# ccchengff/SketchML

Hardware: AMD Instinct MI355X
Metric: device-resident grad encode GB/s (fp32 in) + decode L2 err, 1/2/4/8 GPU (higher is better)
Workload: dtype f32; 1 GPU; north star: 2^28-float dense gradient bucket per GPU, 256 requested bins, encode; n_per_gpu=268435456, bins=256, rotating_buffers=2, parallelism=dp1

## Files before the change

### sketchml_amd/csrc/skml_device.hpp

```cpp
#pragma once
#include <hip/hip_runtime.h>
#include <stdint.h>

#include <type_traits>

#include "skml_internal.h"

namespace skml {

__device__ __forceinline__ uint32_t f2key(uint32_t b) {
    return b ^ ((uint32_t)((int32_t)b >> 31) | 0x80000000u);
}
__device__ __forceinline__ uint32_t key2f(uint32_t k) {
    return k ^ ((k >> 31) ? 0x80000000u : 0xFFFFFFFFu);
}
__device__ __forceinline__ bool is_nan_bits(uint32_t b) { return (b & 0x7FFFFFFFu) > 0x7F800000u; }

typedef _Float16 f16x2_v __attribute__((ext_vector_type(2)));
typedef __bf16 bf16x2_v __attribute__((ext_vector_type(2)));
typedef uint32_t u32x4_v __attribute__((ext_vector_type(4)));
template <typename X>
struct is_lowp : std::integral_constant<bool, std::is_same<X, bf16_t>::value || std::is_same<X, f16_t>::value> {};

template <typename X>
// ... 76 lines not shown
    const uint64_t b = (uint64_t)__double_as_longlong(v);
    const uint32_t lo = lane_xor<M>((uint32_t)b), hi = lane_xor<M>((uint32_t)(b >> 32));
    return __longlong_as_double((long long)(((uint64_t)hi << 32) | lo));
}

__device__ __forceinline__ uint32_t wave_incl_scan_u32(uint32_t v) {
    int x = (int)v;
    x += __builtin_amdgcn_update_dpp(0, x, 0x111, 0xF, 0xF, true);
    x += __builtin_amdgcn_update_dpp(0, x, 0x112, 0xF, 0xF, true);
    x += __builtin_amdgcn_update_dpp(0, x, 0x114, 0xF, 0xF, true);
    x += __builtin_amdgcn_update_dpp(0, x, 0x118, 0xF, 0xF, true);
    x += __builtin_amdgcn_update_dpp(0, x, 0x142, 0xA, 0xF, false);
    x += __builtin_amdgcn_update_dpp(0, x, 0x143, 0xC, 0xF, false);
    return (uint32_t)x;
}

template <int OP>
__device__ __forceinline__ uint32_t dpp_op(uint32_t a, uint32_t b) {
    return OP == 0 ? (a < b ? a : b) : OP == 1 ? (a > b ? a : b) : (a | b);
}
template <int OP>
__device__ __forceinline__ uint32_t wave_reduce_u32_lane63(uint32_t v) {
    constexpr int id = OP == 0 ? -1 : 0;
    int x = (int)v;
    x = (int)dpp_op<OP>((uint32_t)x, (uint32_t)__builtin_amdgcn_update_dpp(id, x, 0x111, 0xF, 0xF, false));
    x = (int)dpp_op<OP>((uint32_t)x, (uint32_t)__builtin_amdgcn_update_dpp(id, x, 0x112, 0xF, 0xF, false));
    x = (int)dpp_op<OP>((uint32_t)x, (uint32_t)__builtin_amdgcn_update_dpp(id, x, 0x114, 0xF, 0xF, false));
    x = (int)dpp_op<OP>((uint32_t)x, (uint32_t)__builtin_amdgcn_update_dpp(id, x, 0x118, 0xF, 0xF, false));
    x = (int)dpp_op<OP>((uint32_t)x, (uint32_t)__builtin_amdgcn_update_dpp(id, x, 0x142, 0xA, 0xF, false));
    x = (int)dpp_op<OP>((uint32_t)x, (uint32_t)__builtin_amdgcn_update_dpp(id, x, 0x143, 0xC, 0xF, false));
    return (uint32_t)x;
}

__device__ __forceinline__ uint32_t elem_fbits(uint32_t k) { return key2f(k); }
__device__ __forceinline__ uint32_t elem_fbits(float f) { return __float_as_uint(f); }
template <typename T>
__device__ __forceinline__ T elem_of_fbits(uint32_t b);
template <>
__device__ __forceinline__ uint32_t elem_of_fbits<uint32_t>(uint32_t b) { return f2key(b); }
template <>
__device__ __forceinline__ float elem_of_fbits<float>(uint32_t b) { return __uint_as_float(b); }
template <typename T>
__device__ __forceinline__ T sel_of(bool upper);
template <>
__device__ __forceinline__ uint32_t sel_of<uint32_t>(bool upper) { return upper ? 0xFFFFFFFFu : 0u; }
template <>
__device__ __forceinline__ float sel_of<float>(bool upper) {
    return __uint_as_float(upper ? 0x7F800000u : 0xFF800000u);
}
template <>
__device__ __forceinline__ double sel_of<double>(bool upper) {
    return __longlong_as_double(upper ? 0x7FF0000000000000LL : (long long)0xFFF0000000000000ULL);
}

template <typename T>
struct Elem {
    using S = float;
    __device__ static __forceinline__ S to_s(uint32_t k) { return __uint_as_float(key2f(k)); }
    __device__ static __forceinline__ uint32_t from_s(S f) { return f2key(__float_as_uint(f)); }
};
template <>
struct Elem<float> {
    using S = float;
    __device__ static __forceinline__ S to_s(float f) { return f; }
    __device__ static __forceinline__ float from_s(S f) { return f; }
};
template <>
struct Elem<double> {
    using S = double;
    __device__ static __forceinline__ S to_s(double d) { return d; }
    __device__ static __forceinline__ double from_s(S d) { return d; }
};

__device__ __forceinline__ void ce(uint32_t& a, uint32_t& b) {
    uint32_t lo = a < b ? a : b;
    uint32_t hi = a < b ? b : a;
    a = lo;
    b = hi;
}
__device__ __forceinline__ void ce(float& a, float& b) {
    float lo, hi;
    asm("v_min_f32 %0, %1, %2" : "=v"(lo) : "v"(a), "v"(b));
    asm("v_max_f32 %0, %1, %2" : "=v"(hi) : "v"(a), "v"(b));
    a = lo;
    b = hi;
// ... 102 lines not shown

template <int R, typename T>
__device__ __forceinline__ void halfclean_regs(T (&v)[R]) {
#pragma unroll
    for (int d = R >> 1; d >= 1; d >>= 1) {
#pragma unroll
        for (int i = 0; i < R; i++) {
            int j = i ^ d;
            if (j > i) ce(v[i], v[j]);
        }
    }
}

__device__ __forceinline__ uint32_t umed3(uint32_t a, uint32_t b, uint32_t c) {
    return min(max(a, b), max(min(a, b), c));
}
__device__ __forceinline__ uint32_t med3(uint32_t a, uint32_t b, uint32_t c) { return umed3(a, b, c); }
__device__ __forceinline__ float med3(float a, float b, float c) { return __builtin_amdgcn_fmed3f(a, b, c); }
__device__ __forceinline__ double med3(double a, double b, double c) {
    double lo, hi;
    asm("v_min_f64 %0, %1, %2" : "=v"(lo) : "v"(a), "v"(b));
    asm("v_max_f64 %0, %1, %2" : "=v"(hi) : "v"(a), "v"(b));
    return __double_as_longlong(c) > 0 ? hi : lo;
}

#ifndef SKML_FLIP_GROUP
#define SKML_FLIP_GROUP 4
#endif
#ifndef SKML_HALF_GROUP
#define SKML_HALF_GROUP 8
#endif
template <int R, int M, typename T>
__device__ __forceinline__ void flip_lanes(T (&v)[R], int lane) {
    const T sel = sel_of<T>((lane & ((M + 1) >> 1)) != 0);
#pragma unroll
    for (int r = 0; r < R / 2; r++) {
        const T pa = lane_xor<M>(v[R - 1 - r]);
        const T pb = lane_xor<M>(v[r]);
        v[r] = med3(v[r], pa, sel);
        v[R - 1 - r] = med3(v[R - 1 - r], pb, sel);
        if ((r & (SKML_FLIP_GROUP - 1)) == SKML_FLIP_GROUP - 1) __builtin_amdgcn_sched_barrier(0);
    }
}

template <int R, int D, typename T>
__device__ __forceinline__ void halfclean_lanes(T (&v)[R], int lane) {
    const T sel = sel_of<T>((lane & D) != 0);
#pragma unroll
    for (int r = 0; r < R; r++) {
        v[r] = med3(v[r], lane_xor<D>(v[r]), sel);
        if ((r & (SKML_HALF_GROUP - 1)) == SKML_HALF_GROUP - 1) __builtin_amdgcn_sched_barrier(0);
    }
}

template <int R, int D, typename T>
__device__ __forceinline__ void halfclean_lanes_down(T (&v)[R], int lane) {
    if constexpr (D >= 1) {
        halfclean_lanes<R, D>(v, lane);
        halfclean_lanes_down<R, D / 2>(v, lane);
    }
}

template <int R, typename T>
__device__ __forceinline__ void merge_group(T (&v)[R], int lane) {
    constexpr int G = 256 / R;
    flip_lanes<R, G - 1>(v, lane);
    halfclean_lanes_down<R, G / 4>(v, lane);
    halfclean_regs<R>(v);
}

template <int R, int S, typename T>
__device__ __forceinline__ void sort_lanes_from(T (&v)[R], int lane) {
    if constexpr (S <= 256) {
        constexpr int M = S / R - 1;
        flip_lanes<R, M>(v, lane);
        halfclean_lanes_down<R, S / R / 4>(v, lane);
        halfclean_regs<R>(v);
        sort_lanes_from<R, S * 2>(v, lane);
    }
}
template <int R, typename T>
__device__ __forceinline__ void sort_group256(T (&v)[R], int lane) {
    sort_regs<R>(v);
    sort_lanes_from<R, 2 * R>(v, lane);
}

template <int R>
__device__ __forceinline__ void compact_regs(const uint32_t (&v)[R], uint32_t (&w)[R / 2], bool odd) {
    const uint32_t m = odd ? 0xFFFFFFFFu : 0u;
#pragma unroll
    for (int j = 0; j < R / 2; j++) w[j] = (v[2 * j + 1] & m) | (v[2 * j] & ~m);
}

template <int R, typename T>
__device__ __forceinline__ void halfclean_regs_compact(T (&v)[R], T (&w)[R / 2], bool odd) {
#pragma unroll
    for (int d = R >> 1; d >= 2; d >>= 1) {
#pragma unroll
        for (int i = 0; i < R; i++) {
            int j = i ^ d;
            if (j > i) ce(v[i], v[j]);
        }
    }
    const T sel = sel_of<T>(odd);
#pragma unroll
    for (int j = 0; j < R / 2; j++) w[j] = med3(v[2 * j], v[2 * j + 1], sel);
}

template <int R, typename T>
__device__ __forceinline__ void merge_group_compact(T (&v)[R], T (&w)[R / 2], int lane, bool odd) {
    constexpr int G = 256 / R;
    flip_lanes<R, G - 1>(v, lane);
    halfclean_lanes_down<R, G / 4>(v, lane);
    halfclean_regs_compact<R>(v, w, odd);
}

template <int R, int S, typename T>
__device__ __forceinline__ void sort_lanes_upto128(T (&v)[R], int lane) {
    if constexpr (S <= 128) {
        constexpr int M = S / R - 1;
        flip_lanes<R, M>(v, lane);
        halfclean_lanes_down<R, S / R / 4>(v, lane);
        halfclean_regs<R>(v);
        sort_lanes_upto128<R, S * 2>(v, lane);
    }
}
template <int R, typename T>
__device__ __forceinline__ void sort_group256_compact(T (&v)[R], T (&w)[R / 2], int lane, bool odd) {
    sort_regs<R>(v);
    sort_lanes_upto128<R, 2 * R>(v, lane);
    merge_group_compact<R>(v, w, lane, odd);
}

__device__ __forceinline__ uint64_t lcg_jump(const uint64_t* __restrict__ tab, uint64_t s,
                                             uint64_t steps) {
#pragma unroll
    for (int lvl = 0; lvl < 4; lvl++) {
        uint32_t b = (uint32_t)(steps >> (8 * lvl)) & 255u;
        if (b) {
            const uint64_t a = tab[(lvl * 256 + b) * 2];
            const uint64_t c = tab[(lvl * 256 + b) * 2 + 1];
            s = (a * s + c) & kLcgMask;
        }
    }
    return s;
}
__device__ __forceinline__ uint32_t lcg_bit(const uint64_t* __restrict__ tab, uint64_t s0,
                                            uint64_t idx) {
    return (uint32_t)(lcg_jump(tab, s0, idx + 1) >> 47) & 1u;
}
__device__ __forceinline__ uint64_t node_bit_index(uint64_t c, int level) {
    return 2 * c - (uint64_t)__popcll(c) + (uint64_t)level;
}

template <typename S>
__device__ __forceinline__ int count_le(const S* run, S x) {
    int lo = 0;
#pragma unroll
    for (int step = 64; step >= 1; step >>= 1)
        if (run[lo + step - 1] <= x) lo += step;
    return lo + (run[lo] <= x ? 1 : 0) * (lo == 127 ? 1 : 0);
}
template <typename S>
__device__ __forceinline__ int count_lt(const S* run, S x) {
    int lo = 0;
#pragma unroll
    for (int step = 64; step >= 1; step >>= 1)
        if (run[lo + step - 1] < x) lo += step;
    return lo + (run[lo] < x ? 1 : 0) * (lo == 127 ? 1 : 0);
}
__device__ __forceinline__ uint32_t tie_pred(float s, float v, uint32_t tie) {
    return (uint32_t)(s < v) | ((uint32_t)(s == v) & tie);
}
__device__ __forceinline__ uint32_t tie_pred(double s, double v, uint32_t tie) {
    return (uint32_t)(s < v) | ((uint32_t)(s == v) & tie);
}
template <typename S>
__device__ __forceinline__ int rank_in_run_pair(const S* a, const S* b, S v, uint32_t tie_a, uint32_t tie_b,
// ... 128 lines not shown
```

### sketchml_amd/csrc/skml_sketch.hip

```cpp
#include <cstdlib>
#include <cstring>
#include <type_traits>

#include "skml_device.hpp"

namespace skml {

__device__ unsigned long long g_prof[32];
#ifdef SKML_PROF_LEAF
__device__ unsigned long long g_leafprof[4 * 65536];
#endif
#ifdef SKML_PROF_SUMMARY
#define SKML_PROF(k)                                      \
    do {                                                  \
        if (threadIdx.x == 0) g_prof[(k)] = wall_clock64(); \
    } while (0)
#else
#define SKML_PROF(k) \
    do {             \
    } while (0)
#endif

constexpr int kWaveFb = 1536;
template <typename S>
// ... 306 lines not shown
#pragma unroll
            for (int j = 0; j < 8; j++) f[j] = src[j * 8 + (lane & 7)];
#pragma unroll
            for (int j = 0; j < 8; j++) {
                const float e4[4] = {f[j].x, f[j].y, f[j].z, f[j].w};
#pragma unroll
                for (int e = 0; e < 4; e++) {
                    zmask |= __ballot(is_class(e4[e], 0x63));
                    v[j * 4 + e] = e4[e];
                }
            }
        }
        if (PARTIAL) zmask &= __ballot(valid);
        uint32_t rfl = 0;
        if (zmask) {
            uint64_t nz = 0, pz = 0, nan = 0;
#pragma unroll
            for (int r = 0; r < 32; r++) {
                nz |= __ballot(is_class(v[r], 0x20));
                pz |= __ballot(is_class(v[r], 0x40));
                nan |= __ballot(is_class(v[r], 0x03));
            }
            if (PARTIAL) {
                nz &= __ballot(valid);
                pz &= __ballot(valid);
                nan &= __ballot(valid);
            }
            rfl = (nz ? 2u : 0u) | (pz ? 4u : 0u) | (nan ? 1u : 0u);
            fl |= rfl;
        }
        const uint64_t start = node_bit_index((uint64_t)c0, 0);
        uint64_t mask;
        {
            const uint64_t s_start = lcg_jump(tab, s0, start + 1);
            const uint64_t s = lane == 0 ? s_start : ((ta * s_start + tc) & kLcgMask);
            mask = __ballot((s >> 47) & 1ull);
        }
        if constexpr (STAGE == 0) {
#pragma unroll
            for (int r = 0; r < 32; r++) acc ^= fold32(v[r]);
            acc ^= (uint32_t)mask;
            continue;
        }
        neg_any = neg_any || (rfl & 2u);
        pos_any = pos_any || (rfl & 4u);
        const bool exact = STAGE == 2 ? false : (neg_any && pos_any);
        auto bit = [&](int level, int64_t last_chunk) -> uint32_t {
            return (uint32_t)(mask >> (node_bit_index((uint64_t)last_chunk, level) - start)) & 1u;
        };

        E w1[16];
        {
            sort_regs_oddeven<32>(v);
            sort_lanes_upto128<32, 64>(v, lane);
            if (valid) {
                const Key k0 = total_key(v[0]), k31 = total_key(v[31]);
                mn = k0 < mn ? k0 : mn;
                mx = k31 > mx ? k31 : mx;
            }
            merge_group_compact<32>(v, w1, lane, bit(0, chunk) != 0);
        }
        const WaveExport<PARTIAL, E> exp{lane, rem, round * kChunksPerWave, roots};
        exp.template at<16>(0, lane >> 3, w1);
        if constexpr (STAGE == 1) {
#pragma unroll
            for (int r = 0; r < 16; r++) acc ^= fold32(w1[r]);
            continue;
        }
        uint32_t ibits = 0;
// ... 19 lines not shown
        if (!(round & 2)) {
            st4[0] = n4[0];
            st4[1] = n4[1];
            continue;
        }
        E n5[2];
        wave_node_merge(st4, n4, n5, lane, bit(5, c0 + 7), exact, wfb);
        if constexpr (PARTIAL)
            if (((rem >> 5) & 1) && round == 3) store_node<2>(n5, lane, roots + (size_t)5 * kK);
        if (!(round & 4)) {
            st5[0] = n5[0];
            st5[1] = n5[1];
            continue;
        }
        wave_node_merge(st5, n5, top, lane, bit(6, c0 + 7), exact, wfb);
    }
    if constexpr (STAGE <= 2) {
        nodes6[(size_t)tile * 64 + lane] = (E)(acc ^ (uint32_t)mn ^ (uint32_t)mx ^ fl);
        return;
    }
    if constexpr (!PARTIAL) {
        if (ubits && tile < upper_node_count(chunks)) {
            int L = kLeafTopLevel + 1;
            int64_t i = tile;
            while (i >= (chunks >> L)) i -= chunks >> L++;
            const uint64_t c = ((uint64_t)(i + 1) << L) - 1;
            if (lane == 0) ubits[tile] = (uint8_t)lcg_bit(tab, s0, node_bit_index(c, L));
        }
    }
    if constexpr (!PARTIAL) {
        store_node<2>(top, lane, nodes6 + (size_t)tile * kK);
        if (((chunks >> 6) & 1) && tile == ((chunks >> 7) << 1)) store_node<2>(top, lane, roots + (size_t)6 * kK);
    }
#pragma unroll
    for (int off = 32; off >= 1; off >>= 1) {
        const Key omn = __shfl_xor(mn, off, 64);
        const Key omx = __shfl_xor(mx, off, 64);
        const uint32_t ofl = (uint32_t)__shfl_xor((int)fl, off, 64);
        mn = omn < mn ? omn : mn;
        mx = omx > mx ? omx : mx;
        fl |= ofl;
    }
    if (lane == 0) {
        typename LeafTypes<E>::Part p;
        p.min_key = mn;
        p.max_key = mx;
        p.flags = fl;
        if constexpr (std::is_same<E, float>::value) p.flags |= (mn < 0x007FFFFFu || mx > 0xFF800000u) ? 1u : 0u;
        p.pad = 0;
        part[tile] = p;
#ifdef SKML_PROF_LEAF
        if (!PARTIAL && tile < 65536) {
            g_leafprof[4 * tile] = prof_t0;
            g_leafprof[4 * tile + 1] = wall_clock64();
            g_leafprof[4 * tile + 2] = __builtin_amdgcn_s_getreg((4 << 0) | (0 << 6) | (31 << 11));
            g_leafprof[4 * tile + 3] = __builtin_amdgcn_s_getreg((20 << 0) | (0 << 6) | (31 << 11));
        }
#endif
    }
}

template <int STAGE, bool PARTIAL = false, typename E = float, typename X = E>
__global__ __launch_bounds__(256, LeafTypes<E>::kMinWaves) void k_leaf2(
    const X* __restrict__ x, int64_t chunks, uint64_t s0, const uint64_t* __restrict__ tab,
    typename LeafTypes<E>::Part* __restrict__ part, E* __restrict__ nodes6, E* __restrict__ roots, int64_t tile0,
    uint8_t* __restrict__ ubits = nullptr) {
    __shared__ E fb[kLeaf2Waves][kWaveFb];
    const int wave = threadIdx.x >> 6;
    leaf2_wave<STAGE, PARTIAL, E, X>(x, chunks, s0, tab, part, nodes6, roots,
                                  tile0 + (int64_t)blockIdx.x * kLeaf2Waves + wave, ubits, fb[wave]);
}

constexpr int kL64Lanes = 4;
constexpr int kL64Chunks = 64 / kL64Lanes;
constexpr int kL64Rounds = kLeafWaveChunks / kL64Chunks;

#ifndef SKML_LEAF64_WAVES
#define SKML_LEAF64_WAVES 4
#endif
#ifndef SKML_LEAF_MIN3DET
#define SKML_LEAF_MIN3DET 1
#endif
#ifndef SKML_LEAF_SPLIT_BELOW
#define SKML_LEAF_SPLIT_BELOW 3072
#endif
struct Leaf64Shared {
    float fb[kLeaf2Waves][kWaveFb];
    float2 stk[kLeaf2Waves][2][64];
    uint32_t wpart[kLeaf2Waves][4];
};
template <bool SPLIT, typename X = float>
__device__ __forceinline__ void leaf64_tile(const X* __restrict__ x, int64_t chunks, uint64_t s0,
                                            const uint64_t* __restrict__ tab, LeafPartial* __restrict__ part,
                                            float* __restrict__ nodes6, float* __restrict__ roots,
                                            uint8_t* __restrict__ ubits, int64_t tile, Leaf64Shared& L) {
    auto& fb = L.fb;
    auto& stk = L.stk;
    auto& wpart = L.wpart;
    const int wave = threadIdx.x >> 6, lane = threadIdx.x & 63;
    const int64_t c_tile = tile * kLeafWaveChunks;
    if (c_tile >= chunks) return;
#ifdef SKML_PROF_LEAF
    const unsigned long long prof_t0 = wall_clock64();
#endif
    float* wfb = fb[wave];
    uint32_t mn = ~0u, mx = 0, fl = 0u;
    bool neg_any = false, pos_any = false;
    float top[2];
    uint64_t split_mask = 0;
    auto run_round = [&](auto ex, int round) -> bool {
        constexpr bool EX = decltype(ex)::value;
        int ln = lane;
        asm volatile("" : "+v"(ln));
        if constexpr (!SPLIT) set_prio_by_progress(round, kL64Rounds);
            const int64_t c0 = c_tile + round * kL64Chunks;
            const int64_t chunk = c0 + (ln >> 2);
            float v[64];
            uint64_t zmask = 0;
            if constexpr (is_lowp<X>::value) {
                const u32x4_v* src = reinterpret_cast<const u32x4_v*>(x + chunk * kChunk);
                u32x4_v f[8];
#pragma unroll
                for (int j = 0; j < 8; j++) f[j] = src[j * kL64Lanes + (ln & 3)];
#pragma unroll
                for (int j = 0; j < 8; j++) widen8<X>(f[j], v + j * 8);
#if SKML_LEAF_MIN3DET
                float za = __builtin_inff(), zb = __builtin_inff();
#pragma unroll
                for (int j = 0; j < 16; j++) {
                    asm("v_minimum3_f32 %0, |%1|, |%2|, %3" : "=v"(za) : "v"(v[j * 4 + 0]), "v"(v[j * 4 + 1]), "v"(za));
                    asm("v_minimum3_f32 %0, |%1|, |%2|, %3" : "=v"(zb) : "v"(v[j * 4 + 2]), "v"(v[j * 4 + 3]), "v"(zb));
                }
// ... 17 lines not shown
                    asm("v_minimum3_f32 %0, |%1|, |%2|, %3" : "=v"(zb) : "v"(f[j].z), "v"(f[j].w), "v"(zb));
                    v[j * 4 + 0] = f[j].x, v[j * 4 + 1] = f[j].y, v[j * 4 + 2] = f[j].z, v[j * 4 + 3] = f[j].w;
                }
                float zm;
                asm("v_minimum3_f32 %0, %1, %2, %2" : "=v"(zm) : "v"(za), "v"(zb));
                zmask = __ballot(!(zm > 0.0f));
#else
#pragma unroll
                for (int j = 0; j < 16; j++) {
                    const float e4[4] = {f[j].x, f[j].y, f[j].z, f[j].w};
#pragma unroll
                    for (int e = 0; e < 4; e++) {
                        zmask |= __ballot(is_class(e4[e], 0x63));
                        v[j * 4 + e] = e4[e];
                    }
                }
#endif
            }
            uint32_t rfl = 0;
            if (zmask) {
                uint64_t nz = 0, pz = 0, nan = 0;
#pragma unroll
                for (int r = 0; r < 64; r++) {
                    nz |= __ballot(is_class(v[r], 0x20));
                    pz |= __ballot(is_class(v[r], 0x40));
                    nan |= __ballot(is_class(v[r], 0x03));
                }
                rfl = (nz ? 2u : 0u) | (pz ? 4u : 0u) | (nan ? 1u : 0u);
                fl |= rfl;
            }
            const uint64_t start = node_bit_index((uint64_t)c0, 0);
            uint64_t mask;
            {
                const uint64_t ta = tab[ln * 2], tc = tab[ln * 2 + 1];
                const uint64_t s_start = lcg_jump(tab, s0, start + 1);
                const uint64_t s = ln == 0 ? s_start : ((ta * s_start + tc) & kLcgMask);
                mask = __ballot((s >> 47) & 1ull);
            }
            neg_any = neg_any || (rfl & 2u);
            pos_any = pos_any || (rfl & 4u);
            if constexpr (!EX) {
                if (neg_any && pos_any) return false;
            }
            const bool exact = EX;
            auto bit = [&](int level, int d) -> uint32_t {
                return (uint32_t)(mask >> (2 * d - __popc((unsigned)d) + level)) & 1u;
            };
            float w1[32];
            sort_regs_oddeven<64>(v);
            sort_lanes_upto128<64, 128>(v, ln);
            {
                const uint32_t k0 = total_key(v[0]), k63 = total_key(v[63]);
                mn = k0 < mn ? k0 : mn;
                mx = k63 > mx ? k63 : mx;
            }
            merge_group_compact<64>(v, w1, ln, bit(0, ln >> 2) != 0);
            float w2[16], w3[8], w4[4], n4[2];
#ifdef SKML_LEAF_ABLATE_TREE
            for (int q = 0; q < 16; q++) w2[q] = fminf(w1[2 * q], w1[2 * q + 1]);
            for (int q = 0; q < 8; q++) w3[q] = w2[2 * q];
            for (int q = 0; q < 4; q++) w4[q] = w3[2 * q];
            n4[0] = w4[0];
            n4[1] = w4[2];
#else
            wave_level<32>(w1, w2, ln, bit(1, 2 * (ln >> 3) + 1), exact, wfb);
            wave_level<16>(w2, w3, ln, bit(2, 4 * (ln >> 4) + 3), exact, wfb);
            wave_level<8>(w3, w4, ln, bit(3, 8 * (ln >> 5) + 7), exact, wfb);
            wave_level<4>(w4, n4, ln, bit(4, 15), exact, wfb);
#endif
            if constexpr (SPLIT) {
                stk[wave][0][ln] = make_float2(n4[0], n4[1]);
                split_mask = mask;
                return true;
            }
            if (!(round & 1)) {
                stk[wave][0][ln] = make_float2(n4[0], n4[1]);
                return true;
            }
            float n5[2];
            {
                const float2 o = stk[wave][0][ln];
                const float st4[2] = {o.x, o.y};
                wave_node_merge(st4, n4, n5, ln, bit(5, 15), exact, wfb);
            }
            if (!(round & 2)) {
                stk[wave][1][ln] = make_float2(n5[0], n5[1]);
                return true;
            }
            const float2 o = stk[wave][1][ln];
            const float st5[2] = {o.x, o.y};
            wave_node_merge(st5, n5, top, ln, bit(6, 15), exact, wfb);
            return true;
    };
    if constexpr (SPLIT) {
        if (!run_round(std::false_type{}, wave)) run_round(std::true_type{}, wave);
#pragma unroll
        for (int off = 32; off >= 1; off >>= 1) {
            const uint32_t omn = __shfl_xor(mn, off, 64);
            const uint32_t omx = __shfl_xor(mx, off, 64);
            const uint32_t ofl = (uint32_t)__shfl_xor((int)fl, off, 64);
            mn = omn < mn ? omn : mn;
            mx = omx > mx ? omx : mx;
            fl |= ofl;
        }
        if (lane == 0) {
            wpart[wave][0] = mn;
            wpart[wave][1] = mx;
            wpart[wave][2] = fl;
        }
        __syncthreads();
        auto zs = [&](int w) { return wpart[w][2] & 6u; };
        const uint32_t b5 = (uint32_t)(split_mask >> 31) & 1u, b6 = (uint32_t)(split_mask >> 32) & 1u;
        if (wave & 1) {
            const uint32_t z = zs(wave - 1) | zs(wave);
            const float2 o = stk[wave - 1][0][lane], m = stk[wave][0][lane];
            const float A[2] = {o.x, o.y}, B[2] = {m.x, m.y};
            float n5[2];
            wave_node_merge(A, B, n5, lane, b5, z == 6u, wfb);
            stk[wave][1][lane] = make_float2(n5[0], n5[1]);
        }
        __syncthreads();
        if (wave != 3) return;
        {
            const uint32_t z = zs(0) | zs(1) | zs(2) | zs(3);
            const float2 o = stk[1][1][lane], m = stk[3][1][lane];
            const float A[2] = {o.x, o.y}, B[2] = {m.x, m.y};
            wave_node_merge(A, B, top, lane, b6, z == 6u, wfb);
        }
        mn = min(min(wpart[0][0], wpart[1][0]), min(wpart[2][0], wpart[3][0]));
        mx = max(max(wpart[0][1], wpart[1][1]), max(wpart[2][1], wpart[3][1]));
        fl = wpart[0][2] | wpart[1][2] | wpart[2][2] | wpart[3][2];
    } else {
        int round = 0;
#pragma unroll 1
        for (; round < kL64Rounds; round++)
            if (!run_round(std::false_type{}, round)) break;
#pragma unroll 1
        for (; round < kL64Rounds; round++) run_round(std::true_type{}, round);
    }
    if (ubits && tile < upper_node_count(chunks)) {
        int L = kLeafTopLevel + 1;
        int64_t i = tile;
        while (i >= (chunks >> L)) i -= chunks >> L++;
        const uint64_t c = ((uint64_t)(i + 1) << L) - 1;
        if (lane == 0) ubits[tile] = (uint8_t)lcg_bit(tab, s0, node_bit_index(c, L));
    }
    store_node<2>(top, lane, nodes6 + (size_t)tile * kK);
    if (((chunks >> 6) & 1) && tile == ((chunks >> 7) << 1)) store_node<2>(top, lane, roots + (size_t)6 * kK);
    if constexpr (!SPLIT) {
#pragma unroll
        for (int off = 32; off >= 1; off >>= 1) {
            const uint32_t omn = __shfl_xor(mn, off, 64);
            const uint32_t omx = __shfl_xor(mx, off, 64);
            const uint32_t ofl = (uint32_t)__shfl_xor((int)fl, off, 64);
            mn = omn < mn ? omn : mn;
            mx = omx > mx ? omx : mx;
            fl |= ofl;
        }
    }
    if (lane == 0) {
        LeafPartial p;
        p.min_key = mn;
        p.max_key = mx;
        p.flags = fl | ((mn < 0x007FFFFFu || mx > 0xFF800000u) ? 1u : 0u);
        p.pad = 0;
        part[tile] = p;
#ifdef SKML_PROF_LEAF
        if (!SPLIT && tile < 65536) {
            g_leafprof[4 * tile] = prof_t0;
            g_leafprof[4 * tile + 1] = wall_clock64();
            g_leafprof[4 * tile + 2] = __builtin_amdgcn_s_getreg((4 << 0) | (0 << 6) | (31 << 11));
            g_leafprof[4 * tile + 3] = __builtin_amdgcn_s_getreg((20 << 0) | (0 << 6) | (31 << 11));
        }
#endif
    }
}

template <int MODE, typename X = float>
__global__ __launch_bounds__(256, SKML_LEAF64_WAVES) void k_leaf64(const X* __restrict__ x, int64_t chunks, uint64_t s0,
                                                   const uint64_t* __restrict__ tab, LeafPartial* __restrict__ part,
                                                   float* __restrict__ nodes6, float* __restrict__ roots,
                                                   uint8_t* __restrict__ ubits, int64_t total_chunks,
                                                   int64_t split_from) {
    __shared__ Leaf64Shared L;
    const int wave = threadIdx.x >> 6;
    int64_t blk = blockIdx.x;
    if (total_chunks > chunks) {
        if (blk == 0) {
            if (wave == 0)
                leaf2_wave<3, true, float, X>(x, total_chunks, s0, tab, part, nodes6, roots, chunks / kLeafWaveChunks,
                                           nullptr, L.fb[0]);
            return;
        }
        blk -= 1;
    }
    if constexpr (MODE == 0) {
        leaf64_tile<false, X>(x, chunks, s0, tab, part, nodes6, roots, ubits, blk * kLeaf2Waves + wave, L);
    } else if constexpr (MODE == 1) {
        leaf64_tile<true, X>(x, chunks, s0, tab, part, nodes6, roots, ubits, blk, L);
    } else {
        const int64_t nwg = split_from / kLeaf2Waves;
        if (blk < nwg) leaf64_tile<false, X>(x, chunks, s0, tab, part, nodes6, roots, ubits, blk * kLeaf2Waves + wave, L);
        else leaf64_tile<true, X>(x, chunks, s0, tab, part, nodes6, roots, ubits, split_from + (blk - nwg), L);
    }
}

template <int STAGE, int MINW = 1>
__global__ __launch_bounds__(512, MINW) void k_leaf(const float* __restrict__ x, int64_t chunks,
                                              uint64_t s0, const uint64_t* __restrict__ tab,
                                              LeafPartial* __restrict__ part,
                                              float* __restrict__ nodes6,
                                              float* __restrict__ roots) {
    __shared__ TileShared sh;
    const int tid = threadIdx.x, wave = tid >> 6, lane = tid & 63;
    const int64_t wg_c0 = (int64_t)blockIdx.x * kLeafChunks;
    const int64_t wave_c0 = wg_c0 + wave * kChunksPerWave;
    const int64_t chunk = wave_c0 + (lane >> 3);
    const int rem = (wg_c0 + kLeafChunks > chunks) ? (int)(chunks - wg_c0) : 0;
// ... 292 lines not shown
    const int64_t base = w > 0 ? wsum[w - 1] : 0;
    *total = wsum[nw - 1];
    __syncthreads();
    return base + x - v;
}

struct SummaryArgs {
    const void* x;
    int64_t n;
    const LeafPartial* part;
    int64_t nparts;
    const float* roots;
    const int64_t* ranks;
    uint8_t* payload;
    double* g_raw;
    QuantLut* lut;
    int req_bins;
    int dedup;
    const float* tail;
    int sharded;
    int64_t n_local;
    const LeafPartial* part_red = nullptr;
    int64_t nred = 0;
    int64_t part_from = 0;
    int xtype = kXF32;
};
__device__ __forceinline__ float load_widen_any(const void* x, int xtype, int64_t i) {
    if (xtype == kXBF16) return load_widen(static_cast<const bf16_t*>(x), i);
    if (xtype == kXF16) return load_widen(static_cast<const f16_t*>(x), i);
    return static_cast<const float*>(x)[i];
}

__device__ void summary_block(const SummaryArgs& a, SummaryShared& S, bool has_pre = false,
                              LeafPartial pre = LeafPartial{0xFFFFFFFFu, 0u, 0u, 0u}) {
    const int t = threadIdx.x, T = blockDim.x;
    skml_dense_header* hdr = reinterpret_cast<skml_dense_header*>(a.payload);
    double* splits = reinterpret_cast<double*>(a.payload + kHeaderBytes);
    const int64_t n = a.n;
    const int64_t chunks = n / kChunk;
    const int tail = (int)(n - chunks * kChunk);
    const void* xt = a.tail ? (const void*)a.tail : a.x;
    const int xt_type = a.tail ? (int)kXF32 : a.xtype;
    const int64_t xt0 = a.tail ? 0 : chunks * kChunk;
    const int req_bins = a.req_bins;
    SKML_PROF(2);

    if (t == 0) {
        S.min_key = 0xFFFFFFFFu;
        S.max_key = 0u;
        S.flags = 0u;
        S.zero = 0x7FFFFFFF;
        int nr = 0, off = 0;
        for (int l = 0; l < kMaxLevels; l++)
            if ((chunks >> l) & 1) {
                S.run_off[nr] = off;
                S.run_lvl[nr] = l;
                nr++;
                off += kK;
            }
        S.run_off[nr] = off;
        S.run_lvl[nr] = -1;
        S.run_off[nr + 1] = off + tail;
        S.nruns = nr + 1;
    }
    __syncthreads();
    {
        uint32_t mn = 0xFFFFFFFFu, mx = 0u, fl = 0u;
// ... 101 lines not shown
            if (r < nfull) rank += run_count_lt(tail_run, tail, v);
            S.sorted[rank] = v;
            S.w[rank] = S.run_lvl[r] < 0 ? 1 : ((int64_t)2 << S.run_lvl[r]);
        }
    }
    __syncthreads();
    SKML_PROF(5);

    {
        const int per = (ns + T - 1) / T;
        const int b0 = min(ns, t * per), b1 = min(ns, b0 + per);
        int64_t loc = 0;
        for (int i = b0; i < b1; i++) loc += S.w[i];
        const int64_t base = block_scan_excl(loc, S.wsum, &S.total);
        int64_t acc = base;
        for (int i = b0; i < b1; i++) {
            const int64_t wv = S.w[i];
            S.w[i] = acc;
            acc += wv;
        }
        if (t == 0) S.w[ns] = S.total;
    }
    __syncthreads();
    SKML_PROF(6);

    const int nsplit_req = req_bins - 1;
    const bool lds_raw = nsplit_req <= kSumMaxRaw;
    double* raw = lds_raw ? S.raw : a.g_raw;
    for (int i = t; i < nsplit_req; i += T) {
        double sp;
        if (ns == 0) {
            sp = __longlong_as_double(0x7FF8000000000000LL);
        } else {
            const int64_t rank = a.ranks[i];
            int lo = 0, hi = ns;
            while (lo + 1 < hi) {
                const int mid = (lo + hi) >> 1;
                if (S.w[mid] <= rank) lo = mid;
                else hi = mid;
            }
            sp = (double)S.sorted[lo];
        }
        raw[i] = sp;
    }
    if (!lds_raw) __threadfence();
    __syncthreads();
    SKML_PROF(7);

    int bin_num;
    {
        const int per = (nsplit_req + T - 1) / T;
        const int b0 = min(nsplit_req, t * per), b1 = min(nsplit_req, b0 + per);
        int64_t loc = 0;
        for (int i = b0; i < b1; i++) loc += (!a.dedup || i == 0 || raw[i] != raw[i - 1]) ? 1 : 0;
        const int64_t base = block_scan_excl(loc, S.wsum, &S.total);
        int64_t o = base;
        int zmin = 0x7FFFFFFF;
        for (int i = b0; i < b1; i++) {
            if (!a.dedup || i == 0 || raw[i] != raw[i - 1]) {
                const double sp = raw[i];
                splits[o] = sp;
                if (o < kMaxSamples) S.smp[o] = (float)sp;
                if (!(sp < 0.0)) zmin = min(zmin, (int)o);
                o++;
            }
        }
        zmin = (int)wave_reduce_u32_lane63<0>((uint32_t)zmin);
// ... 66 lines not shown
        if (level == g && wave == 0 && node == 0) store_node<R>(w, lane, out);
    }
};

template <typename E = float>
__device__ __forceinline__ void merge_group_wg(const MergePass& pass, int wg, const E* __restrict__ src,
                                               E* __restrict__ dst, E* __restrict__ roots, uint64_t s0,
                                               const uint64_t* __restrict__ tab, TileSharedT<E>& sh,
                                               const uint8_t* __restrict__ ubits, int64_t uchunks,
                                               const LeafPartial* __restrict__ part_in = nullptr,
                                               LeafPartial* __restrict__ part_red = nullptr, int prof = -1) {
#ifdef SKML_PROF_SUMMARY
#define SKML_PROF_AT(k)                                                  \
    do {                                                                 \
        if (prof >= 0 && threadIdx.x == 0) g_prof[prof + (k)] = wall_clock64(); \
    } while (0)
#else
#define SKML_PROF_AT(k) \
    do {                \
    } while (0)
#endif
    SKML_PROF_AT(0);
    using T = typename std::conditional<std::is_same<E, double>::value, double, uint32_t>::type;
    const int tid = threadIdx.x, wave = tid >> 6, lane = tid & 63;
    int j = 0;
    while (j + 1 < pass.njobs && wg >= pass.wg_prefix[j + 1]) j++;
    const MergeJob job = pass.job[j];
    const int grp = wg - pass.wg_prefix[j];
    const int g = job.group_log, L = job.level_in;
    const int nodes = 1 << g;
    const int64_t node0 = job.src_node + ((int64_t)grp << g);
    const int64_t chunk0 = job.chunk_base + ((int64_t)grp << (g + L));
    E* out = job.root_level >= 0 ? roots + (size_t)job.root_level * kK : dst + (size_t)(job.dst_node + grp) * kK;
    if (tid == 0) sh.flags = 0u;
    uint32_t bsel = 0;
    {
        int lo = -1, last_node = 0;
        if (lane < 4) lo = 1, last_node = wave * 8 + 2 * lane + 1;
        else if (lane < 6) lo = 2, last_node = wave * 8 + 4 * (lane - 4) + 3;
        else if (lane == 6) lo = 3, last_node = wave * 8 + 7;
        else if (wave == 0 && lane >= 8 && lane < 12) lo = 4, last_node = 16 * (lane - 8) + 15;
        else if (wave == 0 && lane >= 12 && lane < 14) lo = 5, last_node = 32 * (lane - 12) + 31;
        else if (wave == 0 && lane == 14) lo = 6, last_node = 63;
        if (lo > 0) {
            const int lvl = L + lo;
            const int64_t i = ((chunk0 + ((int64_t)(last_node + 1) << L)) >> lvl) - 1;
            const int64_t cnt = upper_node_count(uchunks);
            int64_t idx = upper_level_offset(uchunks, lvl) + i;
            idx = idx < cnt ? idx : cnt - 1;
            bsel = ubits[idx < 0 ? 0 : idx];
        }
    }
    (void)tab;
    (void)s0;
    const bool reduce_parts = part_red && L == kLeafTopLevel && wave == 0;
    LeafPartial tp{0xFFFFFFFFu, 0u, 0u, 0u};
    if (reduce_parts && lane < nodes) tp = part_in[node0 + lane];
    __syncthreads();

    const int nd = wave * 8 + (lane >> 3);
    const bool valid = nd < nodes;
    T w1[16];
    uint32_t fl = 0;
    if constexpr (std::is_same<E, double>::value) {
        const double2* p = reinterpret_cast<const double2*>(src + (size_t)(node0 + (valid ? nd : 0)) * kK) + (lane & 7) * 8;
#pragma unroll
// ... 70 lines not shown
    if (pass.fuse_summary && gridDim.x == 1) SKML_PROF(0);
    merge_group_wg(pass, (int)blockIdx.x, src, dst, roots, s0, tab, U.t, ubits, uchunks, sa.part,
                   const_cast<LeafPartial*>(sa.part_red), blockIdx.x == 0 ? 12 : -1);
    const bool has_next = next.njobs > 0;
    if (!pass.fuse_summary && !has_next) return;

    asm volatile("s_waitcnt vmcnt(0)" ::: "memory");
    __syncthreads();
    if (tid == 0) {
        __builtin_amdgcn_fence(__ATOMIC_RELEASE, "agent");
        asm volatile("s_waitcnt vmcnt(0)" ::: "memory");
        const unsigned old = atomicAdd(done, 1u);
        const int last = old == (unsigned)(pass.wg_prefix[pass.njobs] - 1);
        if (last) {
#ifdef SKML_PROF_SUMMARY
            g_prof[20] = wall_clock64();
#endif
            *done = 0u;
            __builtin_amdgcn_fence(__ATOMIC_ACQUIRE, "agent");
            asm volatile("s_waitcnt vmcnt(0)" ::: "memory");
#ifdef SKML_PROF_SUMMARY
            g_prof[21] = wall_clock64();
#endif
        }
        U.t.is_last = last;
    }
    __syncthreads();
    if (!U.t.is_last) return;
    __syncthreads();
    LeafPartial pre{0xFFFFFFFFu, 0u, 0u, 0u};
    const int64_t npre = sa.nred + (sa.nparts - sa.part_from);
    const bool prefetch = pass.fuse_summary || next.fuse_summary ? npre <= (int64_t)blockDim.x : false;
    if (prefetch && tid < npre) pre = tid < sa.nred ? sa.part_red[tid] : sa.part[sa.part_from + (tid - sa.nred)];
    if (has_next) {
        SKML_PROF(0);
        const int nnext = next.wg_prefix[next.njobs];
        for (int w = 0; w < nnext; w++) {
            if (w) __syncthreads();
            merge_group_wg(next, w, dst, next_dst, roots, s0, tab, U.t, ubits, uchunks, nullptr, nullptr,
                           w == 0 ? 16 : -1);
        }
        asm volatile("s_waitcnt vmcnt(0)" ::: "memory");
        __builtin_amdgcn_fence(__ATOMIC_SEQ_CST, "workgroup");
        __syncthreads();
        if (!next.fuse_summary) return;
    }
    SKML_PROF(1);
    summary_block(sa, U.s, prefetch, pre);
#ifdef SKML_PROF_WARM
    __syncthreads();
    if (threadIdx.x == 0) g_prof[26] = wall_clock64();
    summary_block(sa, U.s);
    __syncthreads();
    if (threadIdx.x == 0) g_prof[27] = wall_clock64();
#endif
}

hipError_t launch_merge_pass(hipStream_t st, const MergePass& pass, const MergePass* next, const float* src,
                             float* dst, float* next_dst, float* roots, uint64_t s0, const uint64_t* jump_tab,
                             unsigned* done, const void* x, int64_t n, const LeafPartial* part, int64_t nparts,
                             const int64_t* ranks, int req_bins, int dedup, void* payload,
                             double* scratch_raw, QuantLut* lut, const uint8_t* ubits, LeafPartial* part_red,
                             int64_t nred, int64_t part_from, int xtype) {
    const int nwg = pass.wg_prefix[pass.njobs];
    if (nwg <= 0) return hipSuccess;
    SummaryArgs a{x, n, part, nparts, roots, ranks, reinterpret_cast<uint8_t*>(payload), scratch_raw,
                  lut, req_bins, dedup};
    a.xtype = xtype;
    a.part_red = part_red;
    a.nred = nred;
    a.part_from = part_from;
    MergePass none;
    if (!next) {
        std::memset(&none, 0, sizeof(none));
        next = &none;
    }
    const int64_t uchunks = (n / kChunk / kLeafWaveChunks) * kLeafWaveChunks;
    hipLaunchKernelGGL(k_merge, dim3(nwg), dim3(512), 0, st, pass, *next, src, dst, next_dst, roots, s0, jump_tab,
                       done, a, ubits, uchunks);
    return hipGetLastError();
}
// ... 297 lines not shown
```

Before: 1858 GB/s.

## Streamline leaf and merge kernels with DPP reductions, scalar LCG jumps, and rank prefetch

```diff
diff --git a/sketchml_amd/csrc/skml_device.hpp b/sketchml_amd/csrc/skml_device.hpp
--- a/sketchml_amd/csrc/skml_device.hpp
+++ b/sketchml_amd/csrc/skml_device.hpp
@@ -132,6 +132,13 @@
     return (uint32_t)x;
 }
 
+__device__ __forceinline__ uint32_t wave_min_u32(uint32_t v) {
+    return (uint32_t)__builtin_amdgcn_readlane((int)wave_reduce_u32_lane63<0>(v), 63);
+}
+__device__ __forceinline__ uint32_t wave_max_u32(uint32_t v) {
+    return (uint32_t)__builtin_amdgcn_readlane((int)wave_reduce_u32_lane63<1>(v), 63);
+}
+
 __device__ __forceinline__ uint32_t elem_fbits(uint32_t k) { return key2f(k); }
 __device__ __forceinline__ uint32_t elem_fbits(float f) { return __float_as_uint(f); }
 template <typename T>
@@ -151,6 +158,14 @@
 template <>
 __device__ __forceinline__ double sel_of<double>(bool upper) {
     return __longlong_as_double(upper ? 0x7FF0000000000000LL : (long long)0xFFF0000000000000ULL);
+}
+__device__ __forceinline__ float sel_of_bit(uint32_t word, uint32_t shl) {
+    return __uint_as_float(((word << shl) & 0x80000000u) ^ 0xFF800000u);
+}
+template <typename T, int D>
+__device__ __forceinline__ T sel_of_lane(int lane) {
+    if constexpr (std::is_same<T, float>::value) return sel_of_bit((uint32_t)lane, 31 - __builtin_ctz(D));
+    else return sel_of<T>((lane & D) != 0);
 }
 
 template <typename T>
@@ -319,7 +334,8 @@
 #endif
 template <int R, int M, typename T>
 __device__ __forceinline__ void flip_lanes(T (&v)[R], int lane) {
-    const T sel = sel_of<T>((lane & ((M + 1) >> 1)) != 0);
+    constexpr int kBit = (M + 1) / 2;
+    const T sel = sel_of_lane<T, kBit>(lane);
 #pragma unroll
     for (int r = 0; r < R / 2; r++) {
         const T pa = lane_xor<M>(v[R - 1 - r]);
@@ -332,7 +348,7 @@
 
 template <int R, int D, typename T>
 __device__ __forceinline__ void halfclean_lanes(T (&v)[R], int lane) {
-    const T sel = sel_of<T>((lane & D) != 0);
+    const T sel = sel_of_lane<T, D>(lane);
 #pragma unroll
     for (int r = 0; r < R; r++) {
         v[r] = med3(v[r], lane_xor<D>(v[r]), sel);
@@ -380,7 +396,7 @@
 }
 
 template <int R, typename T>
-__device__ __forceinline__ void halfclean_regs_compact(T (&v)[R], T (&w)[R / 2], bool odd) {
+__device__ __forceinline__ void halfclean_regs_compact_sel(T (&v)[R], T (&w)[R / 2], T sel) {
 #pragma unroll
     for (int d = R >> 1; d >= 2; d >>= 1) {
 #pragma unroll
@@ -389,17 +405,24 @@
             if (j > i) ce(v[i], v[j]);
         }
     }
-    const T sel = sel_of<T>(odd);
 #pragma unroll
     for (int j = 0; j < R / 2; j++) w[j] = med3(v[2 * j], v[2 * j + 1], sel);
 }
-
-template <int R, typename T>
-__device__ __forceinline__ void merge_group_compact(T (&v)[R], T (&w)[R / 2], int lane, bool odd) {
+template <int R, typename T>
+__device__ __forceinline__ void halfclean_regs_compact(T (&v)[R], T (&w)[R / 2], bool odd) {
+    halfclean_regs_compact_sel<R>(v, w, sel_of<T>(odd));
+}
+
+template <int R, typename T>
+__device__ __forceinline__ void merge_group_compact_sel(T (&v)[R], T (&w)[R / 2], int lane, T sel) {
     constexpr int G = 256 / R;
     flip_lanes<R, G - 1>(v, lane);
     halfclean_lanes_down<R, G / 4>(v, lane);
-    halfclean_regs_compact<R>(v, w, odd);
+    halfclean_regs_compact_sel<R>(v, w, sel);
+}
+template <int R, typename T>
+__device__ __forceinline__ void merge_group_compact(T (&v)[R], T (&w)[R / 2], int lane, bool odd) {
+    merge_group_compact_sel<R>(v, w, lane, sel_of<T>(odd));
 }
 
 template <int R, int S, typename T>
@@ -431,6 +454,29 @@
         }
     }
     return s;
+}
+__device__ __forceinline__ uint64_t lcg_jump_uniform(const uint64_t* __restrict__ tab, uint64_t s, uint64_t steps) {
+    typedef const uint64_t __attribute__((address_space(4))) * ctab_t;
+    const ctab_t t = (ctab_t)(uintptr_t)tab;
+    const uint32_t st = __builtin_amdgcn_readfirstlane((uint32_t)steps);
+    uint64_t a[4], c[4];
+#pragma unroll
+    for (int lvl = 0; lvl < 4; lvl++) {
+        const uint32_t b = (st >> (8 * lvl)) & 255u;
+        a[lvl] = t[(lvl * 256 + b) * 2];
+        c[lvl] = t[(lvl * 256 + b) * 2 + 1];
+    }
+#pragma unroll
+    for (int lvl = 0; lvl < 4; lvl++) s = (a[lvl] * s + c[lvl]) & kLcgMask;
+    return s;
+}
+__device__ __forceinline__ uint32_t lcg_step_next1(uint64_t a, uint64_t c, uint64_t s) {
+    const uint32_t alo = (uint32_t)a, ahi = (uint32_t)(a >> 32), slo = (uint32_t)s, shi = (uint32_t)(s >> 32);
+    const uint64_t p = (uint64_t)alo * slo + c;
+    uint32_t hi = (uint32_t)(p >> 32);
+    asm("v_mad_u32_u24 %0, %1, %2, %0" : "+v"(hi) : "v"(alo), "v"(shi));
+    asm("v_mad_u32_u24 %0, %1, %2, %0" : "+v"(hi) : "v"(ahi), "v"(slo));
+    return (hi >> 15) & 1u;
 }
 __device__ __forceinline__ uint32_t lcg_bit(const uint64_t* __restrict__ tab, uint64_t s0,
                                             uint64_t idx) {
diff --git a/sketchml_amd/csrc/skml_sketch.hip b/sketchml_amd/csrc/skml_sketch.hip
--- a/sketchml_amd/csrc/skml_sketch.hip
+++ b/sketchml_amd/csrc/skml_sketch.hip
@@ -362,9 +362,8 @@
         const uint64_t start = node_bit_index((uint64_t)c0, 0);
         uint64_t mask;
         {
-            const uint64_t s_start = lcg_jump(tab, s0, start + 1);
-            const uint64_t s = lane == 0 ? s_start : ((ta * s_start + tc) & kLcgMask);
-            mask = __ballot((s >> 47) & 1ull);
+            const uint64_t s_start = lcg_jump_uniform(tab, s0, start + 1);
+            mask = __ballot(lcg_step_next1(ta, tc, s_start));
         }
         if constexpr (STAGE == 0) {
 #pragma unroll
@@ -450,14 +449,17 @@
         store_node<2>(top, lane, nodes6 + (size_t)tile * kK);
         if (((chunks >> 6) & 1) && tile == ((chunks >> 7) << 1)) store_node<2>(top, lane, roots + (size_t)6 * kK);
     }
-#pragma unroll
-    for (int off = 32; off >= 1; off >>= 1) {
-        const Key omn = __shfl_xor(mn, off, 64);
-        const Key omx = __shfl_xor(mx, off, 64);
-        const uint32_t ofl = (uint32_t)__shfl_xor((int)fl, off, 64);
-        mn = omn < mn ? omn : mn;
-        mx = omx > mx ? omx : mx;
-        fl |= ofl;
+    if constexpr (std::is_same<Key, uint32_t>::value) {
+        mn = wave_min_u32(mn);
+        mx = wave_max_u32(mx);
+    } else {
+#pragma unroll
+        for (int off = 32; off >= 1; off >>= 1) {
+            const Key omn = __shfl_xor(mn, off, 64);
+            const Key omx = __shfl_xor(mx, off, 64);
+            mn = omn < mn ? omn : mn;
+            mx = omx > mx ? omx : mx;
+        }
     }
     if (lane == 0) {
         typename LeafTypes<E>::Part p;
@@ -484,7 +486,7 @@
     typename LeafTypes<E>::Part* __restrict__ part, E* __restrict__ nodes6, E* __restrict__ roots, int64_t tile0,
     uint8_t* __restrict__ ubits = nullptr) {
     __shared__ E fb[kLeaf2Waves][kWaveFb];
-    const int wave = threadIdx.x >> 6;
+    const int wave = __builtin_amdgcn_readfirstlane((int)(threadIdx.x >> 6));
     leaf2_wave<STAGE, PARTIAL, E, X>(x, chunks, s0, tab, part, nodes6, roots,
                                   tile0 + (int64_t)blockIdx.x * kLeaf2Waves + wave, ubits, fb[wave]);
 }
@@ -515,7 +517,7 @@
     auto& fb = L.fb;
     auto& stk = L.stk;
     auto& wpart = L.wpart;
-    const int wave = threadIdx.x >> 6, lane = threadIdx.x & 63;
+    const int wave = __builtin_amdgcn_readfirstlane((int)(threadIdx.x >> 6)), lane = threadIdx.x & 63;
     const int64_t c_tile = tile * kLeafWaveChunks;
     if (c_tile >= chunks) return;
 #ifdef SKML_PROF_LEAF
@@ -599,10 +601,10 @@
             const uint64_t start = node_bit_index((uint64_t)c0, 0);
             uint64_t mask;
             {
-                const uint64_t ta = tab[ln * 2], tc = tab[ln * 2 + 1];
-                const uint64_t s_start = lcg_jump(tab, s0, start + 1);
-                const uint64_t s = ln == 0 ? s_start : ((ta * s_start + tc) & kLcgMask);
-                mask = __ballot((s >> 47) & 1ull);
+                const ulonglong2 t = reinterpret_cast<const ulonglong2*>(tab)[(uint32_t)ln];
+                const uint64_t ta = t.x, tc = t.y;
+                const uint64_t s_start = lcg_jump_uniform(tab, s0, start + 1);
+                mask = __ballot(lcg_step_next1(ta, tc, s_start));
             }
             neg_any = neg_any || (rfl & 2u);
             pos_any = pos_any || (rfl & 4u);
@@ -612,6 +614,10 @@
             const bool exact = EX;
             auto bit = [&](int level, int d) -> uint32_t {
                 return (uint32_t)(mask >> (2 * d - __popc((unsigned)d) + level)) & 1u;
+            };
+            const uint32_t mask_lo = (uint32_t)mask;
+            auto dsel = [&](int level, int d) -> float {
+                return sel_of_bit(mask_lo, (uint32_t)(31 - level - 2 * d + __popc((unsigned)d)));
             };
             float w1[32];
             sort_regs_oddeven<64>(v);
@@ -621,7 +627,8 @@
                 mn = k0 < mn ? k0 : mn;
                 mx = k63 > mx ? k63 : mx;
             }
-            merge_group_compact<64>(v, w1, ln, bit(0, ln >> 2) != 0);
+            if constexpr (!EX) merge_group_compact_sel<64>(v, w1, ln, dsel(0, ln >> 2));
+            else merge_group_compact<64>(v, w1, ln, bit(0, ln >> 2) != 0);
             float w2[16], w3[8], w4[4], n4[2];
 #ifdef SKML_LEAF_ABLATE_TREE
             for (int q = 0; q < 16; q++) w2[q] = fminf(w1[2 * q], w1[2 * q + 1]);
@@ -630,10 +637,17 @@
             n4[0] = w4[0];
             n4[1] = w4[2];
 #else
-            wave_level<32>(w1, w2, ln, bit(1, 2 * (ln >> 3) + 1), exact, wfb);
-            wave_level<16>(w2, w3, ln, bit(2, 4 * (ln >> 4) + 3), exact, wfb);
-            wave_level<8>(w3, w4, ln, bit(3, 8 * (ln >> 5) + 7), exact, wfb);
-            wave_level<4>(w4, n4, ln, bit(4, 15), exact, wfb);
+            if constexpr (!EX) {
+                merge_group_compact_sel<32>(w1, w2, ln, dsel(1, 2 * (ln >> 3) + 1));
+                merge_group_compact_sel<16>(w2, w3, ln, dsel(2, 4 * (ln >> 4) + 3));
+                merge_group_compact_sel<8>(w3, w4, ln, dsel(3, 8 * (ln >> 5) + 7));
+                merge_group_compact_sel<4>(w4, n4, ln, dsel(4, 15));
+            } else {
+                wave_level<32>(w1, w2, ln, bit(1, 2 * (ln >> 3) + 1), exact, wfb);
+                wave_level<16>(w2, w3, ln, bit(2, 4 * (ln >> 4) + 3), exact, wfb);
+                wave_level<8>(w3, w4, ln, bit(3, 8 * (ln >> 5) + 7), exact, wfb);
+                wave_level<4>(w4, n4, ln, bit(4, 15), exact, wfb);
+            }
 #endif
             if constexpr (SPLIT) {
                 stk[wave][0][ln] = make_float2(n4[0], n4[1]);
@@ -661,15 +675,8 @@
     };
     if constexpr (SPLIT) {
         if (!run_round(std::false_type{}, wave)) run_round(std::true_type{}, wave);
-#pragma unroll
-        for (int off = 32; off >= 1; off >>= 1) {
-            const uint32_t omn = __shfl_xor(mn, off, 64);
-            const uint32_t omx = __shfl_xor(mx, off, 64);
-            const uint32_t ofl = (uint32_t)__shfl_xor((int)fl, off, 64);
-            mn = omn < mn ? omn : mn;
-            mx = omx > mx ? omx : mx;
-            fl |= ofl;
-        }
+        mn = wave_min_u32(mn);
+        mx = wave_max_u32(mx);
         if (lane == 0) {
             wpart[wave][0] = mn;
             wpart[wave][1] = mx;
@@ -715,15 +722,8 @@
     store_node<2>(top, lane, nodes6 + (size_t)tile * kK);
     if (((chunks >> 6) & 1) && tile == ((chunks >> 7) << 1)) store_node<2>(top, lane, roots + (size_t)6 * kK);
     if constexpr (!SPLIT) {
-#pragma unroll
-        for (int off = 32; off >= 1; off >>= 1) {
-            const uint32_t omn = __shfl_xor(mn, off, 64);
-            const uint32_t omx = __shfl_xor(mx, off, 64);
-            const uint32_t ofl = (uint32_t)__shfl_xor((int)fl, off, 64);
-            mn = omn < mn ? omn : mn;
-            mx = omx > mx ? omx : mx;
-            fl |= ofl;
-        }
+        mn = wave_min_u32(mn);
+        mx = wave_max_u32(mx);
     }
     if (lane == 0) {
         LeafPartial p;
@@ -750,7 +750,7 @@
                                                    uint8_t* __restrict__ ubits, int64_t total_chunks,
                                                    int64_t split_from) {
     __shared__ Leaf64Shared L;
-    const int wave = threadIdx.x >> 6;
+    const int wave = __builtin_amdgcn_readfirstlane((int)(threadIdx.x >> 6));
     int64_t blk = blockIdx.x;
     if (total_chunks > chunks) {
         if (blk == 0) {
@@ -1109,7 +1109,8 @@
 }
 
 __device__ void summary_block(const SummaryArgs& a, SummaryShared& S, bool has_pre = false,
-                              LeafPartial pre = LeafPartial{0xFFFFFFFFu, 0u, 0u, 0u}) {
+                              LeafPartial pre = LeafPartial{0xFFFFFFFFu, 0u, 0u, 0u}, bool has_rank = false,
+                              int64_t pre_rank = 0) {
     const int t = threadIdx.x, T = blockDim.x;
     skml_dense_header* hdr = reinterpret_cast<skml_dense_header*>(a.payload);
     double* splits = reinterpret_cast<double*>(a.payload + kHeaderBytes);
@@ -1277,7 +1278,7 @@
         if (ns == 0) {
             sp = __longlong_as_double(0x7FF8000000000000LL);
         } else {
-            const int64_t rank = a.ranks[i];
+            const int64_t rank = has_rank ? pre_rank : a.ranks[i];
             int lo = 0, hi = ns;
             while (lo + 1 < hi) {
                 const int mid = (lo + hi) >> 1;
@@ -1410,6 +1411,45 @@
     const int64_t node0 = job.src_node + ((int64_t)grp << g);
     const int64_t chunk0 = job.chunk_base + ((int64_t)grp << (g + L));
     E* out = job.root_level >= 0 ? roots + (size_t)job.root_level * kK : dst + (size_t)(job.dst_node + grp) * kK;
+    if constexpr (!std::is_same<E, double>::value) {
+        if (g == 2 && !(part_red && L == kLeafTopLevel)) {
+            if (wave != 0) return;
+            uint32_t bsel = 0;
+            if (lane < 3) {
+                const int lo = lane < 2 ? 1 : 2, last_node = lane < 2 ? 2 * lane + 1 : 3;
+                const int lvl = L + lo;
+                const int64_t i = ((chunk0 + ((int64_t)(last_node + 1) << L)) >> lvl) - 1;
+                const int64_t cnt = upper_node_count(uchunks);
+                int64_t idx = upper_level_offset(uchunks, lvl) + i;
+                idx = idx < cnt ? idx : cnt - 1;
+                bsel = ubits[idx < 0 ? 0 : idx];
+            }
+            const float4* p = reinterpret_cast<const float4*>(src + (size_t)(node0 + (lane >> 4)) * kK) + (lane & 15) * 2;
+            T w1[8], w2[4], w3[2];
+            uint32_t fl = 0;
+#pragma unroll
+            for (int q = 0; q < 2; q++) {
+                const float4 f = p[q];
+                const uint32_t b[4] = {__float_as_uint(f.x), __float_as_uint(f.y), __float_as_uint(f.z),
+                                       __float_as_uint(f.w)};
+#pragma unroll
+                for (int e = 0; e < 4; e++) {
+                    fl |= (b[e] == 0x80000000u) ? 2u : 0u;
+                    fl |= (b[e] == 0u) ? 4u : 0u;
+                    w1[q * 4 + e] = f2key(b[e]);
+                }
+            }
+            SKML_PROF_AT(1);
+            const uint32_t bits = (uint32_t)__ballot(bsel != 0);
+            const bool wexact = (__ballot((fl & 2u) != 0) != 0) && (__ballot((fl & 4u) != 0) != 0);
+            wave_level<8>(w1, w2, lane, (bits >> (lane >> 5)) & 1u, wexact, sh.fb[0]);
+            wave_level<4>(w2, w3, lane, (bits >> 2) & 1u, wexact, sh.fb[0]);
+            SKML_PROF_AT(2);
+            store_node<2>(w3, lane, out);
+            SKML_PROF_AT(3);
+            return;
+        }
+    }
     if (tid == 0) sh.flags = 0u;
     uint32_t bsel = 0;
     {
@@ -1546,6 +1586,10 @@
     const int64_t npre = sa.nred + (sa.nparts - sa.part_from);
     const bool prefetch = pass.fuse_summary || next.fuse_summary ? npre <= (int64_t)blockDim.x : false;
     if (prefetch && tid < npre) pre = tid < sa.nred ? sa.part_red[tid] : sa.part[sa.part_from + (tid - sa.nred)];
+    const int nsplit = sa.req_bins - 1;
+    const bool rank_ahead = (pass.fuse_summary || next.fuse_summary) && nsplit <= (int)blockDim.x;
+    int64_t pre_rank = 0;
+    if (rank_ahead && tid < nsplit) pre_rank = sa.ranks[tid];
     if (has_next) {
         SKML_PROF(0);
         const int nnext = next.wg_prefix[next.njobs];
@@ -1560,7 +1604,7 @@
         if (!next.fuse_summary) return;
     }
     SKML_PROF(1);
-    summary_block(sa, U.s, prefetch, pre);
+    summary_block(sa, U.s, prefetch, pre, rank_ahead, pre_rank);
 #ifdef SKML_PROF_WARM
     __syncthreads();
     if (threadIdx.x == 0) g_prof[26] = wall_clock64();
```

Result: faster. 1911 GB/s, median of 6 (+2.9%).
